# ddrainer/FloodPlanet_Code

Measured on AMD Instinct MI355X. Metric: training tiles/sec (256x256x8ch UNet), higher is better.
Workload: dtype bf16; 1 GPU; UNet depth-4 (17.27M params), 8-band 256x256 tiles, batch 16/GPU, fwd+CE(ignore_index=0)+bwd+Adam, train-mode BN; global_batch=16, parallelism=dp1

## Files before the change

floodplanet_code_amd/_lib.py:

```python
from __future__ import annotations

import ctypes as C
import os
from typing import Optional

_HERE = os.path.dirname(os.path.abspath(__file__))
LIB_PATH = os.environ.get("FU_LIB_PATH") or os.path.join(_HERE, "libfloodunet.so")

FU_OK, FU_ERR_INVALID, FU_ERR_HIP, FU_ERR_STATE, FU_ERR_UNSUPPORTED = 0, 1, 2, 3, 4
FU_F32, FU_BF16, FU_F16 = 0, 1, 2
PRECISIONS = {"fp32": FU_F32, "f32": FU_F32, "float32": FU_F32, "bf16": FU_BF16, "bfloat16": FU_BF16,
              "fp16": FU_F16, "f16": FU_F16, "float16": FU_F16, "half": FU_F16}


class FuConfig(C.Structure):
    _fields_ = [
        ("struct_size", C.c_int32),
        ("n_channels", C.c_int32),
        ("n_classes", C.c_int32),
        ("base_channels", C.c_int32),
        ("bilinear", C.c_int32),
        ("max_batch", C.c_int32),
        ("height", C.c_int32),
        ("width", C.c_int32),
# ... 105 lines not shown
    "fu_adam_step_dev": (_i, [_p, _p, _p]),
    "fu_bind_ema_state": (_i, [_p, _p, _p, _p]),
    "fu_adam_ema_step": (_i, [_p, _d, _d, _d, _d, _i64, _d, _d, _p]),
    "fu_adam_ema_scalars": (_i, [_d, _d, _d, _d, _i64, _d, _d, C.POINTER(C.c_float)]),
    "fu_adam_ema_step_dev": (_i, [_p, _p, _p]),
    "fu_zero_grads": (_i, [_p, _p]),
    "fu_stitch_add": (_i, [_p, _i, _p, _p, _i, _i, _i, _i, _i, _i, _p]),
    "fu_stitch_finalize": (_i, [_p, _p, _i, _i, _i, _p, _p]),
    "fu_stitch_add_batch": (_i, [_p, _i, C.POINTER(FuStitchEntry), _p]),
    "fu_eval_confusion": (_i, [_p, _p, _i, _p, _p]),
    "fu_forward_views": (_i, [_p, C.POINTER(_p), C.POINTER(C.c_int32), _i, _i, _i, C.POINTER(C.c_int32), _p, _p]),
    "fu_merge_views": (_i, [_p, _p, _p, _i, _p, _p]),
    "fu_stitch_add_batch_probs": (_i, [_p, _i, C.POINTER(FuStitchEntry), _p, _i, _p]),
    "fu_augment": (_i, [_p, _p, _p, _p, _p, _p, _i, _i, _i, _i, _i64, _p]),
    "fu_scene_crops": (_i, [_p, _i, C.POINTER(FuSceneCrop), _i, _i, _i, _i, _p, _p, _f, _p, _p, _p, _p]),
    "fu_scene_train_tiles": (_i, [_p, _i, C.POINTER(FuSceneTrainEntry), _i, _i, _i, _i, _p, _p, _f, _i64, _i64, _p, _p, _p, _p,
                                  _p]),
    "fu_label_class_counts": (_i, [_p, _i, C.POINTER(FuSceneTrainEntry), _i64, _i, _p, _p]),
    "fu_resize_lanczos4_tiles": (_i, [_p, _i, _i, _i, _i, _p, _p, _p, _p, _i, _i, _i, _p, _p]),
    "fu_assemble_tiles": (_i, [C.POINTER(_p), C.POINTER(C.c_int32), _i, _i, _i, _i, _p, _p, _i, _p, _p, _f, _p, _p, _p, _p]),
    "fu_band_stats_workspace_bytes": (_i64, [_i, _i]),
    "fu_band_stats": (_i, [C.POINTER(_p), C.POINTER(C.c_int32), _i, _i, _i, _i, _p, _p, _i, C.POINTER(FuBandAccum), _p, _i64,
                           _p]),
    "fu_workspace_bytes": (_i64, [_p]),
    "fu_flops_per_tile": (_i, [_p, C.POINTER(C.c_double), C.POINTER(C.c_double)]),
    "fu_profile_enable": (_i, [_p, _i]),
    "fu_test_force_general_conv": (None, [_i]),
    "fu_test_force_lockstep_wgrad": (None, [_i]),
    "fu_test_conv_tile_mode": (None, [_i]),
    "fu_test_bnb_separate": (None, [_i]),
    "fu_test_head_store_g": (None, [_i]),
    "fu_test_force_full_taps": (None, [_i]),
    "fu_test_perturb_bnb_sums": (None, [_f]),
    "fu_test_get_buffer": (_i, [_p, _i, _i, C.POINTER(_p), C.POINTER(_i64)]),
    "fu_set_side_stream": (_i, [_p, _i]),
    "fu_backward_join": (_i, [_p, _p]),
    "fu_backward_fence": (_i, [_p, _p, _p]),
    "fu_dp_unique_id": (_i, [_p]),
    "fu_dp_init": (_i, [_p, _p, _i, _i]),
    "fu_dp_broadcast_state": (_i, [_p, _p]),
    "fu_allreduce_begin": (_i, [_p, _i64, _i64, _p]),
    "fu_allreduce_wait": (_i, [_p, _p]),
    "fu_dp_destroy": (_i, [_p]),
    "fu_set_exact_sync": (_i, [_p, SYNC_HOOK, _p, _i, _p, _i64]),
    "fu_exact_sync_bytes": (_i64, [_p]),
    "fu_profile_read": (_i, [_p, _i, C.POINTER(_i64), C.POINTER(C.c_double), C.POINTER(C.c_double),
                             C.POINTER(C.c_char_p)]),
    "fu_elem_size": (_i, [_i]),
    "fu_op_nchw_to_nhwc": (_i, [_i, _p, _p, _i, _i, _i, _i, _i, _p]),
    "fu_op_nhwc_to_nchw": (_i, [_i, _p, _p, _i, _i, _i, _i, _i, _p]),
    "fu_op_conv3x3_fwd": (_i, [_i, _p, _i, _p, _p, _p, _i, _p, _p, _p, _i, _i, _i, _i, _p, _p, _p]),
    "fu_op_conv3x3_dgrad": (_i, [_i, _p, _i, _p, _p, _i, _p, _i, _i, _i, _i, _p]),
    "fu_op_conv3x3_wgrad": (_i, [_i, _p, _i, _p, _p, _p, _i, _p, _i, _p, _i, _i, _i, _p]),
    "fu_op_conv3x3_dgrad_bnsums": (_i, [_i, _p, _i, _p, _p, _i, _p, _p, _p, _p, _p, _p, _p, _i, _i, _i, _p]),
    "fu_op_head_bwd": (_i, [_i, _p, _p, _p, _p, _p, _i, _i, _i64, _p, _p, _p, _p, _p, _p, _p, _p]),
    "fu_op_bn_bwd": (_i, [_i, _p, _p, _i, _i, _i, _i, _p, _p, _p, _p, _p, _p, _p, _p]),
    "fu_op_maxpool2": (_i, [_i, _p, _p, _p, _p, _i, _i, _i, _i, _p]),
    "fu_op_upsample2": (_i, [_i, _p, _p, _p, _p, _i, _i, _i, _i, _i, _i, _p]),
    "fu_op_upsample2_bwd": (_i, [_i, _p, _p, _i, _i, _i, _i, _i, _i, _p]),
    "fu_op_depth_to_space": (_i, [_i, _p, _p, _i, _i, _i, _i, _i, _i, _p]),
    "fu_op_space_to_depth": (_i, [_i, _p, _p, _i, _i, _i, _i, _i, _i, _p]),
}

_lib: Optional[C.CDLL] = None


def load() -> C.CDLL:
    global _lib
    if _lib is not None:
        return _lib
    if not os.path.exists(LIB_PATH):
        raise RuntimeError(
            f"{LIB_PATH} not found: the HIP extension has not been built. Run "
            "`python -c 'import __graft_entry__ as g; g.build()'` (or `make -C floodplanet_code_amd/csrc`). "
            "There is no CPU / PyTorch fallback for this path.")
    import torch
    lib = C.CDLL(LIB_PATH)
    for name, (res, args) in SIGNATURES.items():
        fn = getattr(lib, name)
        fn.restype = res
        fn.argtypes = args
    _lib = lib
    return lib


def check(status: int) -> None:
    if status != FU_OK:
        msg = load().fu_last_error()
        raise FloodUNetError(status, msg.decode("utf-8", "replace") if msg else "")


def ptr(t) -> Optional[int]:
# ... 2 lines not shown
```

floodplanet_code_amd/csrc/fu_api.hip:

```cpp
#include "../../include/floodunet.h"
#include "fu_common.h"
#include <stdlib.h>

#include <math.h>
#include <string.h>

#include <string>
#include <vector>

using namespace fu;

namespace fu {

int conv3x3_num_stat_tiles(Prec p, int B, int H, int W) {
  return p == PREC_F32 ? conv3x3_num_stat_tiles_f32(B, H, W)
                       : (p == PREC_BF16 ? conv3x3_num_stat_tiles_bf16(B, H, W) : conv3x3_num_stat_tiles_f16(B, H, W));
}
int launch_conv3x3(Prec p, const ConvIn& in, const void* wpk, const float* bias, void* dst0, int D0, void* dst1,
                   int D1, float* stats, int* n_stat_tiles, int B, int H, int W, hipStream_t s) {
  if (p == PREC_F32)
    return launch_conv3x3_f32(in, (const float*)wpk, bias, (float*)dst0, D0, (float*)dst1, D1, stats, n_stat_tiles, B,
                              H, W, s);
  if (p == PREC_BF16)
    return launch_conv3x3_bf16(in, (const bf16_t*)wpk, bias, (bf16_t*)dst0, D0, (bf16_t*)dst1, D1, stats, n_stat_tiles,
// ... 493 lines not shown
  c->p_outb = add_param(c, dscope + "outc.conv.bias", {f.n_classes});
  return 0;
}

int alloc_workspace(fu_ctx* c) {
  const fu_config& f = c->cfg;
  const int B = f.max_batch;
  Arena& A = c->arena;
  const size_t es = c->esize;
  auto act = [&](int level, int C) { return (size_t)B * c->Hs[level] * c->Ws[level] * C * es; };
  for (int e = 0; e < c->nE; ++e) A.want(&c->xin[e], act(0, c->cin_pad0[e]));
  int64_t max_stats = 0, max_bnb = 0, max_slab = 0, max_dbp = 0;
  int max_c = 0;
  for (int i = 0; i < c->nb; ++i) {
    Block& K = c->blk[i];
    for (int j = 0; j < 2; ++j) {
      Conv& v = K.c[j];
      const int H = c->Hs[v.level], W = c->Ws[v.level];
      const int64_t npix = (int64_t)B * H * W;
      A.want(&v.y, act(v.level, v.cout));
      A.want(&v.gy, act(v.level, v.cout));
      A.want(&v.mean, v.cout * sizeof(float));
      A.want(&v.invstd, v.cout * sizeof(float));
      A.want(&v.a, v.cout * sizeof(float));
      A.want(&v.b, v.cout * sizeof(float));
      A.want(&v.coef, v.cout * 2 * sizeof(float));
      A.want(&v.fold_scale, v.cout * sizeof(float));
      A.want(&v.fold_bias, v.cout * sizeof(float));
      A.want(&v.wf, conv3x3_pack_elems(c->prec, v.cin_pad, v.cout) * es);
      if (!(K.role == 0 && j == 0)) A.want(&v.wd, conv3x3_pack_elems(c->prec, v.cin_pad, v.cout) * es);
      max_stats = std::max<int64_t>(max_stats, (int64_t)conv3x3_num_stat_tiles(c->prec, B, H, W) * v.cout * 2);
      max_bnb = std::max<int64_t>(max_bnb, bn_bwd_partial_elems(v.cout, npix));
      max_dbp = std::max<int64_t>(max_dbp, bn_bwd_partial_elems(v.cout, npix) / 2);
      max_slab = std::max<int64_t>(max_slab, conv3x3_wgrad_slab_elems(c->prec, v.cin_pad, v.cout, B, H, W));
      max_c = std::max(max_c, v.cout);
    }
    if (K.kind == BK_DOWN) {
      A.want(&K.pooled, act(K.level, K.c[0].cin_real));
      A.want(&K.g_pooled, act(K.level, K.c[0].cin_real));
    } else if (K.kind == BK_UP) {
      const int clow = K.c[0].cin_real - c->ch[K.skip];
      A.want(&K.up, act(K.level, clow));
      A.want(&K.g_up, act(K.level, clow));
      if (!f.bilinear) {
        const int H = c->Hs[K.level], W = c->Ws[K.level];
        A.want(&K.u, act(K.level, K.ct_cout));
        A.want(&K.g_u, act(K.level, K.ct_cout));
        A.want(&K.ct_w3, (size_t)9 * K.ct_cin * 4 * K.ct_cout * sizeof(float));
        A.want(&K.ct_dw3, (size_t)9 * K.ct_cin * 4 * K.ct_cout * sizeof(float));
        A.want(&K.ct_b4, (size_t)4 * K.ct_cout * sizeof(float));
        A.want(&K.ct_wf, conv3x3_pack_elems(c->prec, K.ct_cin, 4 * K.ct_cout) * es);
        A.want(&K.ct_wd, conv3x3_pack_elems(c->prec, K.ct_cin, 4 * K.ct_cout) * es);
        max_slab = std::max<int64_t>(max_slab, conv3x3_wgrad_slab_elems(c->prec, K.ct_cin, 4 * K.ct_cout, B, H / 2, W / 2));
        max_dbp = std::max<int64_t>(max_dbp, (int64_t)2048 * K.ct_cout);
      }
    }
  }
  for (int l = 0; l < 5 && c->fusion; ++l) {
    Fuse& F = c->fuse[l];
    const int Ccat = c->nE * F.C, H = c->Hs[l], W = c->Ws[l];
    A.want(&F.cat, act(l, Ccat));
    A.want(&F.gcat, act(l, Ccat));
    A.want(&F.y, act(l, F.C));
    A.want(&F.gy, act(l, F.C));
    A.want(&F.w3, (size_t)9 * Ccat * F.C * sizeof(float));
    A.want(&F.dw3, (size_t)9 * Ccat * F.C * sizeof(float));
// ... 235 lines not shown
    if (K.kind == BK_DOWN) {
      Conv& pv = c->blk[i - 1].c[1];
      FU_TRY(launch_maxpool2(c->prec, pv.y, pv.a, pv.b, K.pooled, B, c->Hs[pv.level], c->Ws[pv.level], pv.cout, s));
    } else if (K.kind == BK_UP) {
      const Feat pv = low_feat(c, i);
      const int h = c->Hs[K.level + 1], w = c->Ws[K.level + 1], H = c->Hs[K.level], W = c->Ws[K.level];
      if (c->cfg.bilinear) {
        FU_TRY(launch_upsample2(c->prec, pv.y, pv.a, pv.b, K.up, B, h, w, pv.C, H, W, K.upt, s));
      } else {
        ConvIn lin{pv.y, pv.C, pv.a, pv.b, nullptr, 0, true};
        FU_TRY(launch_conv3x3(c->prec, lin, K.ct_wf, K.ct_b4, K.u, 4 * K.ct_cout, nullptr, 0, nullptr, nullptr, B, h, w, s));
        FU_TRY(launch_depth_to_space(c->prec, K.u, K.up, B, h, w, K.ct_cout, H, W, s));
      }
    }
    FU_TRY(conv_fwd(c, i, 0, B, training, s));
    FU_TRY(conv_fwd(c, i, 1, B, training, s));
  }
  Conv& last = c->blk[c->nb - 1].c[1];
  FU_TRY(launch_head_fwd(c->prec, last.y, last.a, last.b, P(c, c->p_outw), P(c, c->p_outb), f.base_channels,
                         f.n_classes, B, f.height, f.width, c->logits, logits_out, s));
  c->last_batch = B;
  c->view_n = n_views;
  c->view_batch = n_views > 0 ? B / n_views : 0;
  c->view_codes = view_codes;
  c->fwd_training = training;
  c->have_loss = false;
  c->have_up_scale = false;
  return 0;
}

static int g_bnb_separate = 0;
static int g_head_store_g = 0;
static float g_test_perturb_bnb = 1.f;
__global__ void k_scale_floats(float* x, int64_t n, float f) {
  for (int64_t i = (int64_t)blockIdx.x * blockDim.x + threadIdx.x; i < n; i += (int64_t)gridDim.x * blockDim.x) x[i] *= f;
}
int perturb_bnb(float* part, int tiles, int C, hipStream_t s) {
  if (g_test_perturb_bnb == 1.f || tiles <= 0) return 0;
  hipLaunchKernelGGL(k_scale_floats, dim3(256), dim3(256), 0, s, part, (int64_t)tiles * C * 2, g_test_perturb_bnb);
  return hipGetLastError() == hipSuccess ? 0 : FU_ERR_HIP;
}

int backward_conv(fu_ctx* c, int i, int j, int B, hipStream_t s) {
  Block& K = c->blk[i];
  Conv& v = K.c[j];
  const int H = c->Hs[v.level], W = c->Ws[v.level];
  const int64_t npix = (int64_t)B * H * W;
  int ndb = 0;
  const bool side = c->side != nullptr && c->side_mode != 0;
  const int par = c->wg_parity;
  float* dbp = (side && par) ? c->db_part2 : c->db_part;
  if (side && c->wg_pending[par]) FU_HIP_CHECK(hipStreamWaitEvent(s, c->ev_wg[par], 0));
  FU_TRY(launch_bn_bwd(c->prec, v.gy, v.y, v.cout, npix, v.a, v.b, v.mean, v.invstd, P(c, v.p_g), G(c, v.p_g),
                       G(c, v.p_beta), c->bnb_part, v.coef, dbp, &ndb, c->dscratch, s, v.pool_g, B, H, W, v.bnb_tiles,
                       v.head.dl ? &v.head : nullptr));
  v.pool_g = nullptr;
  v.bnb_tiles = 0;
  v.head = HeadGrad{};
  ConvIn in = conv_input(c, i, j);
  const double fl = 2.0 * 9 * v.cin_real * v.cout * (double)B * H * W;
  hipStream_t ws = s;
  if (side) {
    FU_HIP_CHECK(hipEventRecord(c->ev_gy, s));
    FU_HIP_CHECK(hipStreamWaitEvent(c->side, c->ev_gy, 0));
    ws = c->side;
  }
// ... 2 lines not shown
                              G(c, v.p_b), B, H, W, ws));
  if (side) {
    FU_HIP_CHECK(hipEventRecord(c->ev_wg[par], c->side));
    c->wg_pending[par] = true;
    c->wg_parity ^= 1;
  }
  ConvIn din{v.gy, v.cout, nullptr, nullptr, nullptr, 0};
  if (!(K.role == 0 && j == 0)) din.opt.prof = prof_arm(c, FU_K_CONV3X3, fl);
  if (j == 1) {
    Conv& v0 = K.c[0];
    const bool separate = g_bnb_separate != 0;
    int tiles = 0;
    BnbFuse f;
    if (c->prec != PREC_F32 && !c->sync.hook && !separate) {
      f.y = v0.y; f.a = v0.a; f.b = v0.b; f.mean = v0.mean; f.invstd = v0.invstd;
      f.part = c->bnb_part; f.max_elems = c->bnb_cap; f.tiles_out = &tiles;
      din.opt.bnb = &f;
    }
    FU_TRY(launch_conv3x3(c->prec, din, v.wd, nullptr, v0.gy, v0.cout, nullptr, 0, nullptr, nullptr, B, H, W, s));
    v0.bnb_tiles = tiles;
    FU_TRY(perturb_bnb(c->bnb_part, tiles, v0.cout, s));
  } else if (K.kind == BK_DOWN) {
    FU_TRY(launch_conv3x3(c->prec, din, v.wd, nullptr, K.g_pooled, v.cin_real, nullptr, 0, nullptr, nullptr, B, H, W,
                          s));
    Conv& pv = c->blk[i - 1].c[1];
    pv.pool_g = K.g_pooled;
  } else if (K.kind == BK_UP) {
    const Feat sk = level_feat(c, K.skip);
    const Feat pv = low_feat(c, i);
    FU_TRY(launch_conv3x3(c->prec, din, v.wd, nullptr, sk.gy, sk.C, K.g_up, v.cin_real - sk.C, nullptr, nullptr,
                          B, H, W, s));
    const int h = c->Hs[K.level + 1], w = c->Ws[K.level + 1];
    if (c->cfg.bilinear) {
      FU_TRY(launch_upsample2_bwd(c->prec, K.g_up, pv.gy, B, h, w, pv.C, H, W, K.upt, s));
    } else {
      FU_TRY(launch_space_to_depth(c->prec, K.g_up, K.g_u, B, h, w, K.ct_cout, H, W, s));
      int ndbp = 0;
      FU_TRY(launch_channel_partial_sums(c->prec, K.g_u, K.ct_cout, (int64_t)B * h * w * 4, c->db_part, &ndbp, s));
      FU_TRY(launch_colsum_partials(c->db_part, ndbp, K.ct_cout, G(c, K.ct_b), s));
      ConvIn lin{pv.y, pv.C, pv.a, pv.b, nullptr, 0, true};
      FU_TRY(launch_conv3x3_wgrad(c->prec, lin, K.g_u, 4 * K.ct_cout, c->slab, K.ct_dw3, K.ct_cin, nullptr, 0, nullptr, B, h,
                                  w, s));
      FU_TRY(launch_convT_grad_from_w3(K.ct_dw3, K.ct_cin, K.ct_cout, G(c, K.ct_w), s));
      ConvIn gin{K.g_u, 4 * K.ct_cout, nullptr, nullptr, nullptr, 0, true};
      FU_TRY(launch_conv3x3(c->prec, gin, K.ct_wd, nullptr, pv.gy, K.ct_cin, nullptr, 0, nullptr, nullptr, B, h, w, s));
    }
  }
  return 0;
}

int num_backward_blocks(const fu_ctx* c) { return 5 + (c->fusion ? 1 : 0) + 5 * c->nE; }
int backward_block_index(const fu_ctx* c, int block) {
  if (block <= 4) return c->nb - block;
  const int k = block - 5 - (c->fusion ? 1 : 0);
  return 5 * c->nE - 1 - k;
}

int backward_block_impl(fu_ctx* c, int block, const float* dlogits_ext, hipStream_t s, bool join) {
  const fu_config& f = c->cfg;
  const int B = c->last_batch;
  if (block == 0) {
    if (dlogits_ext) {
      FU_TRY(launch_dlogits_from_nchw(dlogits_ext, c->dlogits, f.n_classes, B, f.height, f.width, s));
      c->have_up_scale = false;
    } else {
      FU_REQUIRE(c->have_loss, "fu_backward: no dlogits given and no fu_loss_* call since the last forward");
    }
// ... 929 lines not shown
  if (st == 0) st = launch_upsample2(p, src, bn_a, bn_b, dst, B, H, W, C, outH, outW, t, (hipStream_t)stream);
  (void)hipStreamSynchronize((hipStream_t)stream);
  for (void* q : tmp.extra_allocs) (void)hipFree(q);
  return st;
}

namespace {
int resample_args(const char* who, int precision, Prec* p, const void* a, const void* b, int vec, int B, int H, int W, int C,
                  int outH, int outW) {
  FU_TRY(prec_of(precision, p));
  FU_REQUIRE(a && b, "%s: null argument", who);
  FU_REQUIRE(B > 0 && H > 0 && W > 0 && C > 0, "%s: empty shape (B=%d H=%d W=%d C=%d)", who, B, H, W, C);
  FU_REQUIRE(C % vec == 0, "%s: C=%d is not a multiple of the %d channels of a vector", who, C, vec);
  FU_REQUIRE(outH >= 2 * H && outW >= 2 * W, "%s: target %dx%d smaller than 2x the source %dx%d", who, outH, outW, H, W);
  return 0;
}
}

int fu_op_upsample2_bwd(int precision, const void* g_dst, void* g_src, int B, int H, int W, int C, int outH, int outW,
                        fu_stream stream) {
  Prec p;
  FU_TRY(resample_args("fu_op_upsample2_bwd", precision, &p, g_dst, g_src, 16 / fu_elem_size(precision), B, H, W, C, outH,
                       outW));
  fu_ctx tmp;
  UpTables t;
  int st = build_up_tables(&tmp, H, W, &t);
  if (st == 0) st = launch_upsample2_bwd(p, g_dst, g_src, B, H, W, C, outH, outW, t, (hipStream_t)stream);
  const hipError_t e = hipStreamSynchronize((hipStream_t)stream);
  for (void* q : tmp.extra_allocs) (void)hipFree(q);
  if (st == 0 && e != hipSuccess) { set_error("fu_op_upsample2_bwd: %s", hipGetErrorString(e)); return FU_ERR_HIP; }
  return st;
}

int fu_op_depth_to_space(int precision, const void* y4, void* up, int B, int h, int w, int C, int outH, int outW,
                         fu_stream stream) {
  Prec p;
  FU_TRY(resample_args("fu_op_depth_to_space", precision, &p, y4, up, 4, B, h, w, C, outH, outW));
  FU_TRY(launch_depth_to_space(p, y4, up, B, h, w, C, outH, outW, (hipStream_t)stream));
  FU_HIP_CHECK(hipStreamSynchronize((hipStream_t)stream));
  return FU_OK;
}

int fu_op_space_to_depth(int precision, const void* gup, void* g4, int B, int h, int w, int C, int outH, int outW,
                         fu_stream stream) {
  Prec p;
  FU_TRY(resample_args("fu_op_space_to_depth", precision, &p, gup, g4, 4, B, h, w, C, outH, outW));
  FU_TRY(launch_space_to_depth(p, gup, g4, B, h, w, C, outH, outW, (hipStream_t)stream));
  FU_HIP_CHECK(hipStreamSynchronize((hipStream_t)stream));
  return FU_OK;
}

namespace {
int collapse_partials(const float* part, int nTiles, int C, float* s1, float* s2, hipStream_t s) {
  hipLaunchKernelGGL(k_stats_collapse, dim3(ceil_div(C, 64)), dim3(64), 0, s, part, nTiles, C, s1, s2);
  hipError_t e = hipGetLastError();
  if (e != hipSuccess) { set_error("collapse launch failed: %s", hipGetErrorString(e)); return FU_ERR_HIP; }
  return 0;
}
}

int fu_op_conv3x3_dgrad_bnsums(int precision, const void* dy, int Cout, const float* w_oihw, void* dx, int C0,
                               const void* y, const float* bn_a, const float* bn_b, const float* mean,
                               const float* invstd, float* sum_gm, float* sum_gmx, int B, int H, int W,
                               fu_stream stream) {
  Prec p; FU_TRY(prec_of(precision, &p));
  FU_REQUIRE(p != PREC_F32, "fu_op_conv3x3_dgrad_bnsums: 16-bit precisions only (fp32 keeps the separate reduce pass)");
// ... 64 lines not shown
  FU_TRY(coef.get((size_t)C * 2 * sizeof(float)));
  FU_TRY(dbp.get((size_t)bn_bwd_partial_elems(C, npix) * sizeof(float)));
  FU_TRY(scr.get((size_t)reduce_scratch_elems(std::max(C, 64)) * sizeof(double)));
  int ndb = 0;
  FU_TRY(launch_bn_bwd(p, g, y, C, npix, bn_a, bn_b, mean, invstd, nullptr, dgamma, dbeta, (float*)part.p,
                       (float*)coef.p, (float*)dbp.p, &ndb, (double*)scr.p, s, g_pool, B, H, W, 0));
  FU_HIP_CHECK(hipStreamSynchronize(s));
  return FU_OK;
}

int fu_test_get_buffer(fu_ctx* c, int block, int which, void** ptr, int64_t* elems) {
  FU_REQUIRE(c && ptr && elems, "fu_test_get_buffer: null argument");
  FU_REQUIRE(block >= 0 && block < c->nb, "fu_test_get_buffer: block %d outside 0..%d", block, c->nb - 1);
  const Block& K = c->blk[block];
  const int B = c->cfg.max_batch;
  auto act = [&](int level, int C) { return (int64_t)B * c->Hs[level] * c->Ws[level] * C; };
  switch (which) {
    case 0: *ptr = K.c[0].y; *elems = act(K.c[0].level, K.c[0].cout); break;
    case 1: *ptr = K.c[0].gy; *elems = act(K.c[0].level, K.c[0].cout); break;
    case 2: *ptr = K.c[1].y; *elems = act(K.c[1].level, K.c[1].cout); break;
    case 3: *ptr = K.c[1].gy; *elems = act(K.c[1].level, K.c[1].cout); break;
    case 4: *ptr = K.g_pooled; *elems = K.kind == BK_DOWN ? act(K.level, K.c[0].cin_real) : 0; break;
    case 5: *ptr = K.g_up; *elems = K.kind == BK_UP ? act(K.level, K.c[0].cin_real - c->ch[K.skip]) : 0; break;
    default: set_error("fu_test_get_buffer: which must be 0..5"); return FU_ERR_INVALID;
  }
  return FU_OK;
}

}

extern "C" void fu_test_bnb_separate(int on) { g_bnb_separate = on ? 1 : 0; }
extern "C" void fu_test_head_store_g(int on) { g_head_store_g = on ? 1 : 0; }
extern "C" void fu_test_perturb_bnb_sums(float factor) { g_test_perturb_bnb = factor; }
```

floodplanet_code_amd/csrc/fu_common.h:

```cpp
#pragma once
#include <hip/hip_runtime.h>
#include <stdint.h>
#include <stdio.h>
#include <string>

struct fu_stitch_entry;
struct fu_scene_crop;
struct fu_scene_train_entry;

namespace fu {

typedef unsigned short bf16_t;
struct f16_t { unsigned short v; };

enum Prec { PREC_F32 = 0, PREC_BF16 = 1, PREC_F16 = 2 };

template <typename F> auto dispatch_prec(Prec p, F&& f) {
  if (p == PREC_F32) return f(float{});
  if (p == PREC_BF16) return f(bf16_t{});
  return f(f16_t{});
}

void set_error(const char* fmt, ...);
const char* get_error();
// ... 300 lines not shown
                        int src_channels = 0, int src_channel_offset = 0);
int launch_nhwc_to_nchw(Prec p, const void* src, float* dst, int B, int C, int H, int W, int c_pad, hipStream_t s);
struct SrcList { const float* p[8]; int c[8]; int coff[9]; int n; };
int launch_gather_nchw_to_nhwc(Prec p, const SrcList& S, void* dst, int B, int C, int H, int W, int c_pad, int ch_off,
                               hipStream_t s);
int launch_gather_views_nchw_to_nhwc(Prec p, const SrcList& S, void* dst, int B, int n_views, unsigned codes, int C, int H,
                                     int W, int c_pad, int ch_off, hipStream_t s);

int launch_bn_finalize(const float* partials, int nTiles, int C, int64_t count, const float* conv_bias,
                       const float* gamma, const float* beta, float eps, float momentum, float* mean, float* invstd,
                       float* a, float* b, float* running_mean, float* running_var, int64_t* nbt, double* dscratch,
                       hipStream_t s);
static inline int64_t reduce_scratch_elems(int C) { return (int64_t)32 * C * 2; }
int64_t bn_bwd_partial_elems(int C, int64_t npix);
int launch_bn_bwd(Prec p, void* g, const void* y, int C, int64_t npix, const float* a, const float* b,
                  const float* mean, const float* invstd, const float* gamma, float* dgamma, float* dbeta,
                  float* partials, float* coef, float* db_partials, int* n_db_partials, double* dscratch,
                  hipStream_t s, const void* g_pool = nullptr, int B = 0, int H = 0, int W = 0, int ext_partials = 0,
                  const HeadGrad* head = nullptr);

int launch_maxpool2(Prec p, const void* src, const float* a, const float* b, void* dst, int B, int H, int W, int C,
                    hipStream_t s);
struct UpTables {
  const int* y_i0; const int* y_i1; const float* y_w1;
  const int* x_i0; const int* x_i1; const float* x_w1;
  const int* yb_o; const float* yb_w;
  const int* xb_o; const float* xb_w;
  float scale_y, scale_x;
};
static constexpr int UP_BWD_MAX = 6;
int launch_upsample2(Prec p, const void* src, const float* a, const float* b, void* dst, int B, int H, int W, int C,
                     int outH, int outW, const UpTables& t, hipStream_t s);
int launch_upsample2_bwd(Prec p, const void* g_dst, void* g_src, int B, int H, int W, int C, int outH, int outW,
                         const UpTables& t, hipStream_t s);

int launch_depth_to_space(Prec p, const void* y4, void* up, int B, int h, int w, int C, int outH, int outW, hipStream_t s);
int launch_space_to_depth(Prec p, const void* gup, void* g4, int B, int h, int w, int C, int outH, int outW, hipStream_t s);
int launch_colsum_partials(const float* partials, int n, int C, float* out, hipStream_t s);
int launch_channel_partial_sums(Prec p, const void* g, int C, int64_t npix, float* partials, int* n_partials,
                                hipStream_t s);
int launch_convT_to_w3(const float* w, const float* b, int Cin, int Cout, float* w3, float* bias4, hipStream_t s);
int launch_convT_grad_from_w3(const float* dw3, int Cin, int Cout, float* dw, hipStream_t s);
int launch_copy_channels(Prec p, const void* src, int srcC, int src_off, const float* a, const float* b, void* dst,
                         int dstC, int dst_off, int C, int64_t npix, hipStream_t s);
int launch_center_to_w3(const float* w, int64_t n, float* w3, hipStream_t s);
int launch_center_from_w3(const float* dw3, int64_t n, float* dw, hipStream_t s);

int launch_head_fwd(Prec p, const void* y, const float* a, const float* b, const float* w, const float* bias, int C,
                    int ncls, int B, int H, int W, float* logits_nhwc, float* logits_nchw, hipStream_t s);
static constexpr int HEAD_MAX_CLS = 8;
static constexpr int LOSS_PART_FLOATS = 4 * 1024;
struct CeWeighting {
  const float* class_weight;
  float c_nll, c_smooth;
  float* weight_sum_dev;
  float* weight_sum_out;
};
int launch_ce_loss(const float* logits_nhwc, const int64_t* target, int ncls, int ignore_index, int64_t npix,
                   const CeWeighting* cw, float* partials, float* loss_out, int64_t* n_valid_dev,
                   int64_t* confusion_accum, int64_t* n_valid_out, unsigned long long* conf_tmp ,
                   hipStream_t s);
int launch_ce_grad(const float* logits_nhwc, const int64_t* target, int ncls, int ignore_index, int64_t npix,
                   const CeWeighting* cw, const int64_t* n_valid_dev, float* dlogits_nhwc, hipStream_t s);
int launch_bce_dice(const float* logits_nhwc, const int64_t* target, int ncls, int ignore_index, int64_t npix,
                    float dice_w, float* partials, float* coef, float* loss_out, int64_t* n_valid_dev,
                    float* dlogits_nhwc, hipStream_t s);
int launch_dlogits_from_nchw(const float* dlogits_nchw, float* dlogits_nhwc, int ncls, int B, int H, int W,
// ... 52 lines not shown
```

floodplanet_code_amd/csrc/fu_elementwise.hip:

```cpp
#include "fu_common.h"

#include <stdarg.h>

namespace fu {

thread_local const SyncDesc* g_sync = nullptr;
thread_local const float* g_grad_unscale = nullptr;

int sync_sum_over_ranks(void* payload, int64_t n_elems, bool is_double, hipStream_t s) {
  const SyncDesc* d = g_sync;
  if (!d || !d->hook || d->world <= 1) return 0;
  const size_t bytes = (size_t)n_elems * (is_double ? 8 : 4);
  FU_REQUIRE((int64_t)bytes <= d->xbytes, "exact sync: exchange buffer too small (%zu > %lld bytes)", bytes,
             (long long)d->xbytes);
  FU_HIP_CHECK(hipMemcpyAsync(d->xbuf, payload, bytes, hipMemcpyDeviceToDevice, s));
  if (d->hook(d->user, n_elems, is_double ? 1 : 0) != 0) {
    set_error("exact sync: the all-reduce hook failed");
    return 3;
  }
  FU_HIP_CHECK(hipMemcpyAsync(payload, d->xbuf, bytes, hipMemcpyDeviceToDevice, s));
  return 0;
}

static thread_local char g_err[1024] = "";
void set_error(const char* fmt, ...) {
  va_list ap;
  va_start(ap, fmt);
  vsnprintf(g_err, sizeof(g_err), fmt, ap);
  va_end(ap);
}
const char* get_error() { return g_err; }

template <typename T>
__global__ void k_nchw_to_nhwc(const float* __restrict__ src, T* __restrict__ dst, int C, int HW, int cpad,
                               int64_t total, int srcC) {
// ... 852 lines not shown
  constexpr int V = VecIO<T>::V;
  const int item = blockIdx.x * 256 + threadIdx.x;
  if (item >= W * CV) return;
  const int ix = fast_div(item, CV, rcpCV), cv = item - ix * CV;
  const int iy = blockIdx.y, bb = blockIdx.z;
  float acc[V];
#pragma unroll
  for (int j = 0; j < V; ++j) acc[j] = 0.f;
  const T* base = gdst + (size_t)bb * outH * outW * C + cv * V;
  int xo[UP_BWD_MAX];
  float xw[UP_BWD_MAX];
#pragma unroll
  for (int jx = 0; jx < UP_BWD_MAX; ++jx) { xo[jx] = t.xb_o[ix * UP_BWD_MAX + jx]; xw[jx] = t.xb_w[ix * UP_BWD_MAX + jx]; }
  for (int jy = 0; jy < UP_BWD_MAX; ++jy) {
    const int oy = t.yb_o[iy * UP_BWD_MAX + jy];
    if (oy < 0) break;
    const float wy = t.yb_w[iy * UP_BWD_MAX + jy];
    const T* rowp = base + (size_t)(oy + py0) * outW * C;
#pragma unroll
    for (int jx = 0; jx < UP_BWD_MAX; ++jx) {
      if (__builtin_amdgcn_ballot_w64(xo[jx] >= 0) == 0) break;
      if (xo[jx] >= 0) {
        const float w = wy * xw[jx];
        float gv[V];
        VecIO<T>::load(rowp + (size_t)(xo[jx] + px0) * C, gv);
#pragma unroll
        for (int j = 0; j < V; ++j) acc[j] += w * gv[j];
      }
    }
  }
  VecIO<T>::store(gsrc + ((size_t)(bb * H + iy) * W + ix) * C + cv * V, acc);
}

int launch_upsample2(Prec p, const void* src, const float* a, const float* b, void* dst, int B, int H, int W, int C,
                     int outH, int outW, const UpTables& t, hipStream_t s) {
  FU_REQUIRE(outH >= 2 * H && outW >= 2 * W, "upsample: target smaller than 2x source");
  const int py0 = (outH - 2 * H) / 2, px0 = (outW - 2 * W) / 2;
  return dispatch_prec(p, [&](auto tag) {
    using T = decltype(tag);
    dim3 g; int CV; unsigned rcp;
    FU_REQUIRE(row_grid<T>(C, outW, outH, B, &g, &CV, &rcp), "upsample: unsupported shape (C=%d H=%d B=%d)", C, outH, B);
    if ((int64_t)g.x * ceil_div(outH, 4) * B >= 2048) {
      g.y = ceil_div(outH, 4);
      hipLaunchKernelGGL((k_upsample2<T, 4>), g, dim3(256), 0, s, (const T*)src, a, b, (T*)dst, H, W, C, outH, outW, py0, px0,
                         t, CV, rcp);
    } else {
      hipLaunchKernelGGL((k_upsample2<T, 1>), g, dim3(256), 0, s, (const T*)src, a, b, (T*)dst, H, W, C, outH, outW, py0, px0,
                         t, CV, rcp);
    }
    FU_LAUNCH_CHECK();
    return 0;
  });
}

int launch_upsample2_bwd(Prec p, const void* g_dst, void* g_src, int B, int H, int W, int C, int outH, int outW,
                         const UpTables& t, hipStream_t s) {
  FU_REQUIRE(outH >= 2 * H && outW >= 2 * W, "upsample_bwd: target smaller than 2x source");
  const int py0 = (outH - 2 * H) / 2, px0 = (outW - 2 * W) / 2;
  return dispatch_prec(p, [&](auto tag) {
    using T = decltype(tag);
    dim3 g; int CV; unsigned rcp;
    FU_REQUIRE(row_grid<T>(C, W, H, B, &g, &CV, &rcp), "upsample_bwd: unsupported shape (C=%d H=%d B=%d)", C, H, B);
    hipLaunchKernelGGL(k_upsample2_bwd<T>, g, dim3(256), 0, s, (const T*)g_dst, (T*)g_src, H, W, C, outH, outW, py0, px0, t,
                       CV, rcp);
    FU_LAUNCH_CHECK();
    return 0;
  });
}

template <typename T>
__global__ void k_depth_to_space(const T* __restrict__ y4, T* __restrict__ up, int h, int w, int C, int outH, int outW,
                                 int py0, int px0, int64_t total) {
  const int CV = C >> 2;
  for (int64_t idx = (int64_t)blockIdx.x * blockDim.x + threadIdx.x; idx < total;
       idx += (int64_t)gridDim.x * blockDim.x) {
    const int cv = (int)(idx % CV);
    int64_t r = idx / CV;
    const int ox = (int)(r % outW); r /= outW;
    const int oy = (int)(r % outH);
    const int64_t bb = r / outH;
    float o[4] = {0, 0, 0, 0};
    const int uy = oy - py0, ux = ox - px0;
    if (uy >= 0 && uy < 2 * h && ux >= 0 && ux < 2 * w) {
      const int ph = (uy & 1) * 2 + (ux & 1);
      ElemIO<T>::load4(y4 + (((bb * h + (uy >> 1)) * w + (ux >> 1)) * 4 + ph) * (int64_t)C + cv * 4, o);
    }
    ElemIO<T>::store4(up + idx * 4, o);
  }
}
template <typename T>
__global__ void k_space_to_depth(const T* __restrict__ gup, T* __restrict__ g4, int h, int w, int C, int outH, int outW,
                                 int py0, int px0, int64_t total) {
  const int CV = C >> 2;
  for (int64_t idx = (int64_t)blockIdx.x * blockDim.x + threadIdx.x; idx < total;
       idx += (int64_t)gridDim.x * blockDim.x) {
    const int cv = (int)(idx % CV);
    int64_t r = idx / CV;
    const int ph = (int)(r & 3); r >>= 2;
// ... 486 lines not shown
```

include/floodunet.h:

```cpp
#ifndef FLOODUNET_H_
#define FLOODUNET_H_

#include <stddef.h>
#include <stdint.h>

#ifdef __cplusplus
extern "C" {
#endif

#define FU_ABI_VERSION 5
#define FU_MAX_ENCODERS 6

typedef struct fu_ctx fu_ctx;
typedef void* fu_stream;

enum fu_status {
  FU_OK = 0,
  FU_ERR_INVALID = 1,
  FU_ERR_HIP = 2,
  FU_ERR_STATE = 3,
  FU_ERR_UNSUPPORTED = 4
};

enum fu_precision {
// ... 156 lines not shown
} fu_stitch_entry;
int fu_stitch_add_batch(fu_ctx* ctx, int n, const fu_stitch_entry* entries, fu_stream stream);

enum { FU_VIEW_HFLIP = 1, FU_VIEW_VFLIP = 2, FU_VIEW_TRANSPOSE = 4 };
int fu_forward_views(fu_ctx* ctx, const float* const* srcs, const int32_t* src_channels, int n_src, int batch,
                     int n_views, const int32_t* codes, float* logits_out, fu_stream stream);
int fu_merge_views(fu_ctx* ctx, float* probs_out, const int64_t* target, int ignore_index, int64_t* counts_out,
                   fu_stream stream);
int fu_stitch_add_batch_probs(fu_ctx* ctx, int n, const fu_stitch_entry* entries, const float* probs, int batch,
                              fu_stream stream);

int fu_eval_confusion(fu_ctx* ctx, const int64_t* target, int ignore_index, int64_t* counts_out, fu_stream stream);

int64_t fu_workspace_bytes(const fu_ctx* ctx);
int fu_flops_per_tile(const fu_ctx* ctx, double* fwd, double* train);

enum fu_kernel_class {
  FU_K_CONV3X3 = 0,
  FU_K_WGRAD = 1,
  FU_K_NUM = 2
};
int fu_profile_enable(fu_ctx* ctx, int enable);
int fu_profile_read(fu_ctx* ctx, int kernel_class, int64_t* launches, double* total_ms, double* total_flops,
                    const char** kernel_name);

void fu_test_force_general_conv(int on);
void fu_test_force_lockstep_wgrad(int on);
void fu_test_conv_tile_mode(int mode);
void fu_test_bnb_separate(int on);
void fu_test_head_store_g(int on);
void fu_test_force_full_taps(int on);

void fu_test_perturb_bnb_sums(float factor);
int fu_test_get_buffer(fu_ctx* ctx, int block, int which, void** ptr, int64_t* elems);

int fu_elem_size(int precision);
int fu_op_nchw_to_nhwc(int precision, const float* src, void* dst, int B, int C, int H, int W, int c_pad,
                       fu_stream stream);
int fu_op_nhwc_to_nchw(int precision, const void* src, float* dst, int B, int C, int H, int W, int c_pad,
                       fu_stream stream);
int fu_op_conv3x3_fwd(int precision, const void* src0, int C0, const float* bn_a0, const float* bn_b0,
                      const void* src1, int C1, const float* w_oihw, const float* bias, void* y, int Cout, int B,
                      int H, int W, float* stats_sum, float* stats_sqsum, fu_stream stream);
int fu_op_conv3x3_dgrad(int precision, const void* dy, int Cout, const float* w_oihw, void* dx0, int C0, void* dx1,
                        int C1, int B, int H, int W, fu_stream stream);
int fu_op_conv3x3_wgrad(int precision, const void* src0, int C0, const float* bn_a0, const float* bn_b0,
                        const void* src1, int C1, const void* dy, int Cout, float* dw_oihw, int B, int H, int W,
                        fu_stream stream);
int fu_op_maxpool2(int precision, const void* src, const float* bn_a, const float* bn_b, void* dst, int B, int H,
                   int W, int C, fu_stream stream);
int fu_op_upsample2(int precision, const void* src, const float* bn_a, const float* bn_b, void* dst, int B, int H,
                    int W, int C, int outH, int outW, fu_stream stream);
int fu_op_upsample2_bwd(int precision, const void* g_dst, void* g_src, int B, int H, int W, int C, int outH, int outW,
                        fu_stream stream);
int fu_op_depth_to_space(int precision, const void* y4, void* up, int B, int h, int w, int C, int outH, int outW,
                         fu_stream stream);
int fu_op_space_to_depth(int precision, const void* gup, void* g4, int B, int h, int w, int C, int outH, int outW,
                         fu_stream stream);

int fu_op_conv3x3_dgrad_bnsums(int precision, const void* dy, int Cout, const float* w_oihw, void* dx, int C0,
                               const void* y, const float* bn_a, const float* bn_b, const float* mean,
                               const float* invstd, float* sum_gm, float* sum_gmx, int B, int H, int W,
                               fu_stream stream);
int fu_op_head_bwd(int precision, const float* dlogits_nhwc, const void* y, const float* bn_a, const float* bn_b,
                   const float* w, int C, int ncls, int64_t npix, void* g, float* dw, float* db, const float* mean,
                   const float* invstd, float* sum_gm, float* sum_gmx, fu_stream stream);
int fu_op_bn_bwd(int precision, void* g, const void* y, int C, int B, int H, int W, const float* bn_a,
                 const float* bn_b, const float* mean, const float* invstd, const void* g_pool, float* dgamma,
                 float* dbeta, fu_stream stream);

#ifdef __cplusplus
}
#endif
#endif
```

Before: 3258 tiles/s.

## Tile bilinear upsample backward through LDS and fuse BN-backward partial sums

Replaces the per-row gather kernel for bilinear upsample backward with a tiled kernel that stages the needed output-gradient patch in LDS and reuses it across four input rows. In bf16/fp16, it also computes the BN-backward partial sums (sum of masked gradient and gradient times normalized activation) for the preceding block's conv in the same pass and writes per-tile partials. This removes the separate reduction over that activation later, at the cost of a more complex kernel, extra LDS use and a larger partial buffer.

```diff
diff --git a/floodplanet_code_amd/_lib.py b/floodplanet_code_amd/_lib.py
--- a/floodplanet_code_amd/_lib.py
+++ b/floodplanet_code_amd/_lib.py
@@ -161,6 +161,8 @@
     "fu_test_head_store_g": (None, [_i]),
     "fu_test_force_full_taps": (None, [_i]),
     "fu_test_perturb_bnb_sums": (None, [_f]),
+    "fu_test_upsample_bwd_gather": (None, [_i]),
+    "fu_test_upsample_bwd_fused": (_i, [_i]),
     "fu_test_get_buffer": (_i, [_p, _i, _i, C.POINTER(_p), C.POINTER(_i64)]),
     "fu_set_side_stream": (_i, [_p, _i]),
     "fu_backward_join": (_i, [_p, _p]),
@@ -187,6 +189,7 @@
     "fu_op_maxpool2": (_i, [_i, _p, _p, _p, _p, _i, _i, _i, _i, _p]),
     "fu_op_upsample2": (_i, [_i, _p, _p, _p, _p, _i, _i, _i, _i, _i, _i, _p]),
     "fu_op_upsample2_bwd": (_i, [_i, _p, _p, _i, _i, _i, _i, _i, _i, _p]),
+    "fu_op_upsample2_bwd_sums": (_i, [_i, _p, _p, _i, _i, _i, _i, _i, _i, _p, _p, _p, _p, _p, _p, _i64, C.POINTER(_i), _p]),
     "fu_op_depth_to_space": (_i, [_i, _p, _p, _i, _i, _i, _i, _i, _i, _p]),
     "fu_op_space_to_depth": (_i, [_i, _p, _p, _i, _i, _i, _i, _i, _i, _p]),
 }
diff --git a/floodplanet_code_amd/csrc/fu_api.hip b/floodplanet_code_amd/csrc/fu_api.hip
--- a/floodplanet_code_amd/csrc/fu_api.hip
+++ b/floodplanet_code_amd/csrc/fu_api.hip
@@ -549,6 +549,7 @@
       max_stats = std::max<int64_t>(max_stats, (int64_t)conv3x3_num_stat_tiles(c->prec, B, H, W) * v.cout * 2);
       max_bnb = std::max<int64_t>(max_bnb, bn_bwd_partial_elems(v.cout, npix));
       max_dbp = std::max<int64_t>(max_dbp, bn_bwd_partial_elems(v.cout, npix) / 2);
+      if (j == 1 && f.bilinear) max_bnb = std::max<int64_t>(max_bnb, upsample2_bwd_partial_elems(c->prec, B, H, W, v.cout));
       max_slab = std::max<int64_t>(max_slab, conv3x3_wgrad_slab_elems(c->prec, v.cin_pad, v.cout, B, H, W));
       max_c = std::max(max_c, v.cout);
     }
@@ -850,6 +851,7 @@
 static int g_bnb_separate = 0;
 static int g_head_store_g = 0;
 static float g_test_perturb_bnb = 1.f;
+static int g_upbwd_fused_launches = 0;
 __global__ void k_scale_floats(float* x, int64_t n, float f) {
   for (int64_t i = (int64_t)blockIdx.x * blockDim.x + threadIdx.x; i < n; i += (int64_t)gridDim.x * blockDim.x) x[i] *= f;
 }
@@ -918,7 +920,20 @@
                           B, H, W, s));
     const int h = c->Hs[K.level + 1], w = c->Ws[K.level + 1];
     if (c->cfg.bilinear) {
-      FU_TRY(launch_upsample2_bwd(c->prec, K.g_up, pv.gy, B, h, w, pv.C, H, W, K.upt, s));
+      Conv* lv = (c->fusion && i == 5 * c->nE) ? nullptr : &c->blk[i - 1].c[1];
+      int tiles = 0;
+      BnbFuse f;
+      const bool want = lv && c->prec != PREC_F32 && !c->sync.hook && !g_bnb_separate;
+      if (want) {
+        f.y = lv->y; f.a = lv->a; f.b = lv->b; f.mean = lv->mean; f.invstd = lv->invstd;
+        f.part = c->bnb_part; f.max_elems = c->bnb_cap; f.tiles_out = &tiles;
+      }
+      FU_TRY(launch_upsample2_bwd(c->prec, K.g_up, pv.gy, B, h, w, pv.C, H, W, K.upt, s, want ? &f : nullptr));
+      if (lv) {
+        lv->bnb_tiles = tiles;
+        FU_TRY(perturb_bnb(c->bnb_part, tiles, lv->cout, s));
+        if (tiles > 0) ++g_upbwd_fused_launches;
+      }
     } else {
       FU_TRY(launch_space_to_depth(c->prec, K.g_up, K.g_u, B, h, w, K.ct_cout, H, W, s));
       int ndbp = 0;
@@ -1914,6 +1929,30 @@
   return st;
 }
 
+int fu_op_upsample2_bwd_sums(int precision, const void* g_dst, void* g_src, int B, int H, int W, int C, int outH, int outW,
+                             const void* y, const float* bn_a, const float* bn_b, const float* mean, const float* invstd,
+                             float* part, int64_t max_elems, int* tiles_out, fu_stream stream) {
+  Prec p;
+  FU_TRY(resample_args("fu_op_upsample2_bwd_sums", precision, &p, g_dst, g_src, 16 / fu_elem_size(precision), B, H, W, C, outH,
+                       outW));
+  FU_REQUIRE(y && bn_a && bn_b && mean && invstd && part && tiles_out, "fu_op_upsample2_bwd_sums: null argument");
+  FU_REQUIRE(max_elems >= 0, "fu_op_upsample2_bwd_sums: negative max_elems");
+  fu_ctx tmp;
+  UpTables t;
+  BnbFuse f;
+  f.y = y; f.a = bn_a; f.b = bn_b; f.mean = mean; f.invstd = invstd;
+  f.part = part; f.max_elems = max_elems; f.tiles_out = tiles_out;
+  const int before = *tiles_out;
+  hipStream_t s = (hipStream_t)stream;
+  int st = build_up_tables(&tmp, H, W, &t);
+  if (st == 0) st = launch_upsample2_bwd(p, g_dst, g_src, B, H, W, C, outH, outW, t, s, &f);
+  if (st == 0 && *tiles_out != before) st = perturb_bnb(part, *tiles_out, C, s);
+  const hipError_t e = hipStreamSynchronize(s);
+  for (void* q : tmp.extra_allocs) (void)hipFree(q);
+  if (st == 0 && e != hipSuccess) { set_error("fu_op_upsample2_bwd_sums: %s", hipGetErrorString(e)); return FU_ERR_HIP; }
+  return st;
+}
+
 int fu_op_depth_to_space(int precision, const void* y4, void* up, int B, int h, int w, int C, int outH, int outW,
                          fu_stream stream) {
   Prec p;
@@ -2044,3 +2083,9 @@
 extern "C" void fu_test_bnb_separate(int on) { g_bnb_separate = on ? 1 : 0; }
 extern "C" void fu_test_head_store_g(int on) { g_head_store_g = on ? 1 : 0; }
 extern "C" void fu_test_perturb_bnb_sums(float factor) { g_test_perturb_bnb = factor; }
+extern "C" void fu_test_upsample_bwd_gather(int on) { fu::g_upsample_bwd_gather = on ? 1 : 0; }
+extern "C" int fu_test_upsample_bwd_fused(int reset) {
+  const int n = g_upbwd_fused_launches;
+  if (reset) g_upbwd_fused_launches = 0;
+  return n;
+}
diff --git a/floodplanet_code_amd/csrc/fu_common.h b/floodplanet_code_amd/csrc/fu_common.h
--- a/floodplanet_code_amd/csrc/fu_common.h
+++ b/floodplanet_code_amd/csrc/fu_common.h
@@ -356,7 +356,9 @@
 int launch_upsample2(Prec p, const void* src, const float* a, const float* b, void* dst, int B, int H, int W, int C,
                      int outH, int outW, const UpTables& t, hipStream_t s);
 int launch_upsample2_bwd(Prec p, const void* g_dst, void* g_src, int B, int H, int W, int C, int outH, int outW,
-                         const UpTables& t, hipStream_t s);
+                         const UpTables& t, hipStream_t s, const BnbFuse* fuse = nullptr);
+int64_t upsample2_bwd_partial_elems(Prec p, int B, int H, int W, int C);
+extern int g_upsample_bwd_gather;
 
 int launch_depth_to_space(Prec p, const void* y4, void* up, int B, int h, int w, int C, int outH, int outW, hipStream_t s);
 int launch_space_to_depth(Prec p, const void* gup, void* g4, int B, int h, int w, int C, int outH, int outW, hipStream_t s);
diff --git a/floodplanet_code_amd/csrc/fu_elementwise.hip b/floodplanet_code_amd/csrc/fu_elementwise.hip
--- a/floodplanet_code_amd/csrc/fu_elementwise.hip
+++ b/floodplanet_code_amd/csrc/fu_elementwise.hip
@@ -1,6 +1,7 @@
 #include "fu_common.h"
 
 #include <stdarg.h>
+#include <algorithm>
 
 namespace fu {
 
@@ -919,6 +920,157 @@
   VecIO<T>::store(gsrc + ((size_t)(bb * H + iy) * W + ix) * C + cv * V, acc);
 }
 
+static constexpr int UPB_R = 4;
+static constexpr int UPB_NR = 12;
+static constexpr int UPB_ROWCAP = 160;
+static constexpr int UPB_MAX_ROWS = 2048;
+struct UpBnb { const void* y; const float *a, *b, *mean, *invstd; float* part; };
+
+template <typename T, bool BNB>
+__global__ __launch_bounds__(256) void k_upsample2_bwd_tile(const T* __restrict__ gdst, T* __restrict__ gsrc, int H, int W,
+                                                            int C, int outH, int outW, int py0, int px0, UpTables t, int lg,
+                                                            int nTx, int tiles_y, UpBnb f) {
+  constexpr int V = VecIO<T>::V;
+  __shared__ uint4 patch[UPB_NR * UPB_ROWCAP];
+  const int tid = threadIdx.x;
+  const int CVg = 1 << lg, Wt = 64 >> lg;
+  const int cg = blockIdx.x / nTx, tx = blockIdx.x - cg * nTx;
+  const int bb = blockIdx.z;
+  const int v = tid & (CVg - 1), lx = (tid & 63) >> lg;
+  const int r = __builtin_amdgcn_readfirstlane(tid >> 6);
+  const int ix = tx * Wt + lx;
+  const bool xok = ix < W;
+  const int c0 = (cg * CVg + v) * V;
+  int xo[UP_BWD_MAX];
+  float xw[UP_BWD_MAX];
+  int xlo = 0x7fffffff, xhi = -1;
+#pragma unroll
+  for (int jx = 0; jx < UP_BWD_MAX; ++jx) {
+    xo[jx] = xok ? t.xb_o[ix * UP_BWD_MAX + jx] : -1;
+    xw[jx] = xok ? t.xb_w[ix * UP_BWD_MAX + jx] : 0.f;
+    if (xo[jx] >= 0) { xlo = min(xlo, xo[jx]); xhi = max(xhi, xo[jx]); }
+  }
+#pragma unroll
+  for (int off = 32; off > 0; off >>= 1) {
+    xlo = min(xlo, __shfl_xor(xlo, off, 64));
+    xhi = max(xhi, __shfl_xor(xhi, off, 64));
+  }
+  xlo = __builtin_amdgcn_readfirstlane(xlo);
+  xhi = __builtin_amdgcn_readfirstlane(xhi);
+  const int rowlen = (xhi - xlo + 1) << lg;
+  float av[V], bv[V], s1[V], s2[V];
+  if (BNB) {
+    load_coef<V>(f.a, f.b, c0, av, bv);
+#pragma unroll
+    for (int j = 0; j < V; ++j) { s1[j] = 0.f; s2[j] = 0.f; }
+  }
+  for (int tt = 0; tt < tiles_y; ++tt) {
+    const int iy0 = (blockIdx.y * tiles_y + tt) * UPB_R;
+    if (iy0 >= H) break;
+    int ylo = 0x7fffffff, yhi = -1;
+    for (int rr = 0; rr < UPB_R && iy0 + rr < H; ++rr)
+      for (int jy = 0; jy < UP_BWD_MAX; ++jy) {
+        const int o = t.yb_o[(iy0 + rr) * UP_BWD_MAX + jy];
+        if (o >= 0) { ylo = min(ylo, o); yhi = max(yhi, o); }
+      }
+    const int nrow = yhi - ylo + 1;
+    const bool in_lds = nrow > 0 && nrow <= UPB_NR && rowlen > 0 && rowlen <= UPB_ROWCAP;
+    const int iy = iy0 + r;
+    const bool active = xok && iy < H;
+    const size_t so = ((size_t)(bb * H + (active ? iy : 0)) * W + (active ? ix : 0)) * C + c0;
+    float yv[V];
+    if (BNB) VecIO<T>::load(reinterpret_cast<const T*>(f.y) + so, yv);
+    if (in_lds) {
+      constexpr int NLD = (UPB_NR * UPB_ROWCAP + 255) / 256;
+      uint4 tmp[NLD];
+#pragma unroll
+      for (int k = 0; k < NLD; ++k) {
+        const int idx = tid + k * 256;
+        const int pr = idx / UPB_ROWCAP, j = idx - pr * UPB_ROWCAP;
+        const bool ok = pr < nrow && j < rowlen;
+        const int col = j >> lg, vv = j & (CVg - 1);
+        const T* p = gdst + ((size_t)(bb * outH + ylo + pr + py0) * outW + (xlo + col + px0)) * C + (cg * CVg + vv) * V;
+        tmp[k] = ok ? *reinterpret_cast<const uint4*>(p) : make_uint4(0u, 0u, 0u, 0u);
+      }
+#pragma unroll
+      for (int k = 0; k < NLD; ++k) {
+        const int idx = tid + k * 256;
+        const int pr = idx / UPB_ROWCAP, j = idx - pr * UPB_ROWCAP;
+        if (pr < nrow && j < rowlen) patch[idx] = tmp[k];
+      }
+    }
+    __syncthreads();
+    if (active) {
+      float acc[V];
+#pragma unroll
+      for (int j = 0; j < V; ++j) acc[j] = 0.f;
+      const T* base = gdst + (size_t)bb * outH * outW * C + c0;
+      for (int jy = 0; jy < UP_BWD_MAX; ++jy) {
+        const int oy = t.yb_o[iy * UP_BWD_MAX + jy];
+        if (oy < 0) break;
+        const float wy = t.yb_w[iy * UP_BWD_MAX + jy];
+        const T* rowp = base + (size_t)(oy + py0) * outW * C;
+        const int lrow = (oy - ylo) * UPB_ROWCAP + v;
+#pragma unroll
+        for (int jx = 0; jx < UP_BWD_MAX; ++jx) {
+          if (__builtin_amdgcn_ballot_w64(xo[jx] >= 0) == 0) break;
+          if (xo[jx] >= 0) {
+            const float w = wy * xw[jx];
+            float gv[V];
+            if (in_lds) VecIO<T>::load(reinterpret_cast<const T*>(&patch[lrow + ((xo[jx] - xlo) << lg)]), gv);
+            else VecIO<T>::load(rowp + (size_t)(xo[jx] + px0) * C, gv);
+#pragma unroll
+            for (int j = 0; j < V; ++j) acc[j] += w * gv[j];
+          }
+        }
+      }
+      VecIO<T>::store(gsrc + so, acc);
+      if (BNB) {
+#pragma unroll
+        for (int j = 0; j < V; ++j) {
+          const float gm = bn_act_pre(av[j], yv[j], bv[j]) > 0.f ? acc[j] : 0.f;
+          s1[j] += gm;
+          s2[j] = fmaf(gm, yv[j], s2[j]);
+        }
+      }
+    }
+    __syncthreads();
+  }
+  if (BNB) {
+    float* red = reinterpret_cast<float*>(patch);
+    const int NCH = CVg * V;
+#pragma unroll
+    for (int j = 0; j < V; ++j) {
+#pragma unroll
+      for (int off = 32; off > 0; off >>= 1) {
+        if (off >= CVg) {
+          s1[j] += __shfl_xor(s1[j], off, 64);
+          s2[j] += __shfl_xor(s2[j], off, 64);
+        }
+      }
+    }
+    if ((tid & 63) < CVg) {
+#pragma unroll
+      for (int j = 0; j < V; ++j) {
+        red[(r * NCH + v * V + j) * 2 + 0] = s1[j];
+        red[(r * NCH + v * V + j) * 2 + 1] = s2[j];
+      }
+    }
+    __syncthreads();
+    if (tid < NCH) {
+      float u1 = 0.f, u2 = 0.f;
+#pragma unroll
+      for (int m = 0; m < 4; ++m) { u1 += red[(m * NCH + tid) * 2 + 0]; u2 += red[(m * NCH + tid) * 2 + 1]; }
+      const int c = cg * NCH + tid;
+      const int64_t row = ((int64_t)bb * gridDim.y + blockIdx.y) * nTx + tx;
+      const float is = f.invstd[c];
+      float* o = f.part + (row * C + c) * 2;
+      o[0] = u1;
+      o[1] = fmaf(is, u2, -(f.mean[c] * is) * u1);
+    }
+  }
+}
+
 int launch_upsample2(Prec p, const void* src, const float* a, const float* b, void* dst, int B, int H, int W, int C,
                      int outH, int outW, const UpTables& t, hipStream_t s) {
   FU_REQUIRE(outH >= 2 * H && outW >= 2 * W, "upsample: target smaller than 2x source");
@@ -940,17 +1092,67 @@
   });
 }
 
+int g_upsample_bwd_gather = 0;
+
+namespace {
+struct UpBwdGeom { int lg, nTx, nCg, tiles_y, gy; int64_t rows; };
+bool upb_geom(Prec p, int B, int H, int W, int C, UpBwdGeom* g) {
+  const int V = p == PREC_F32 ? 4 : 8;
+  if (B < 1 || H < 1 || W < 1 || C < V || C % V != 0 || B > 65535) return false;
+  const int CV = C / V;
+  int lg = 0;
+  while (lg < 3 && (CV & ((2 << lg) - 1)) == 0) ++lg;
+  const int nTy = ceil_div(H, UPB_R);
+  g->lg = lg;
+  g->nTx = ceil_div(W, 64 >> lg);
+  g->nCg = CV >> lg;
+  int ty = 1;
+  while (ty < nTy && (int64_t)B * ceil_div(nTy, ty) * g->nTx > UPB_MAX_ROWS) ++ty;
+  g->tiles_y = ty;
+  g->gy = ceil_div(nTy, ty);
+  g->rows = (int64_t)B * g->gy * g->nTx;
+  return g->gy <= 65535 && (int64_t)g->nTx * g->nCg < ((int64_t)1 << 31);
+}
+}
+
+int64_t upsample2_bwd_partial_elems(Prec p, int B, int H, int W, int C) {
+  UpBwdGeom g;
+  if (p == PREC_F32 || !upb_geom(p, B, H, W, C, &g)) return 0;
+  return std::min<int64_t>(UPB_MAX_ROWS, (int64_t)B * ceil_div(H, UPB_R) * g.nTx) * C * 2;
+}
+
 int launch_upsample2_bwd(Prec p, const void* g_dst, void* g_src, int B, int H, int W, int C, int outH, int outW,
-                         const UpTables& t, hipStream_t s) {
+                         const UpTables& t, hipStream_t s, const BnbFuse* fuse) {
   FU_REQUIRE(outH >= 2 * H && outW >= 2 * W, "upsample_bwd: target smaller than 2x source");
   const int py0 = (outH - 2 * H) / 2, px0 = (outW - 2 * W) / 2;
+  UpBwdGeom G;
+  const bool tiled = !g_upsample_bwd_gather && upb_geom(p, B, H, W, C, &G);
   return dispatch_prec(p, [&](auto tag) {
     using T = decltype(tag);
-    dim3 g; int CV; unsigned rcp;
-    FU_REQUIRE(row_grid<T>(C, W, H, B, &g, &CV, &rcp), "upsample_bwd: unsupported shape (C=%d H=%d B=%d)", C, H, B);
-    hipLaunchKernelGGL(k_upsample2_bwd<T>, g, dim3(256), 0, s, (const T*)g_dst, (T*)g_src, H, W, C, outH, outW, py0, px0, t,
-                       CV, rcp);
+    if (!tiled) {
+      dim3 g; int CV; unsigned rcp;
+      FU_REQUIRE(row_grid<T>(C, W, H, B, &g, &CV, &rcp), "upsample_bwd: unsupported shape (C=%d H=%d B=%d)", C, H, B);
+      hipLaunchKernelGGL(k_upsample2_bwd<T>, g, dim3(256), 0, s, (const T*)g_dst, (T*)g_src, H, W, C, outH, outW, py0, px0, t,
+                         CV, rcp);
+      FU_LAUNCH_CHECK();
+      return 0;
+    }
+    const dim3 g(G.nTx * G.nCg, G.gy, B);
+    const bool sums = fuse && fuse->tiles_out && fuse->part && fuse->y && sizeof(T) == 2 && G.rows <= UPB_MAX_ROWS &&
+                      G.rows * C * 2 <= fuse->max_elems;
+    if constexpr (sizeof(T) == 2) {
+      if (sums) {
+        const UpBnb f{fuse->y, fuse->a, fuse->b, fuse->mean, fuse->invstd, fuse->part};
+        hipLaunchKernelGGL((k_upsample2_bwd_tile<T, true>), g, dim3(256), 0, s, (const T*)g_dst, (T*)g_src, H, W, C, outH,
+                           outW, py0, px0, t, G.lg, G.nTx, G.tiles_y, f);
+      }
+    }
+    if (!sums) {
+      hipLaunchKernelGGL((k_upsample2_bwd_tile<T, false>), g, dim3(256), 0, s, (const T*)g_dst, (T*)g_src, H, W, C, outH,
+                         outW, py0, px0, t, G.lg, G.nTx, G.tiles_y, UpBnb{});
+    }
     FU_LAUNCH_CHECK();
+    if (sums) *fuse->tiles_out = (int)G.rows;
     return 0;
   });
 }
diff --git a/include/floodunet.h b/include/floodunet.h
--- a/include/floodunet.h
+++ b/include/floodunet.h
@@ -212,6 +212,8 @@
 void fu_test_force_full_taps(int on);
 
 void fu_test_perturb_bnb_sums(float factor);
+void fu_test_upsample_bwd_gather(int on);
+int fu_test_upsample_bwd_fused(int reset);
 int fu_test_get_buffer(fu_ctx* ctx, int block, int which, void** ptr, int64_t* elems);
 
 int fu_elem_size(int precision);
@@ -233,6 +235,9 @@
                     int W, int C, int outH, int outW, fu_stream stream);
 int fu_op_upsample2_bwd(int precision, const void* g_dst, void* g_src, int B, int H, int W, int C, int outH, int outW,
                         fu_stream stream);
+int fu_op_upsample2_bwd_sums(int precision, const void* g_dst, void* g_src, int B, int H, int W, int C, int outH, int outW,
+                             const void* y, const float* bn_a, const float* bn_b, const float* mean, const float* invstd,
+                             float* part, int64_t max_elems, int* tiles_out, fu_stream stream);
 int fu_op_depth_to_space(int precision, const void* y4, void* up, int B, int h, int w, int C, int outH, int outW,
                          fu_stream stream);
 int fu_op_space_to_depth(int precision, const void* gup, void* g4, int B, int h, int w, int C, int outH, int outW,
```

After: 3250 tiles/s. Within noise of the previous version (-0.2%).
